# az16/MD_RDM

Measured on AMD Instinct MI355X. Metric: depth-maps/sec NYU 228x304 batch=16 fwd+bwd, higher is better.
Workload: dtype f32 (bf16x6-split 1x1 forward of dense_e2/e3, bf16x3-split gradient GEMMs of dense_e2/e3/e4); 1 GPU; NYU-v2 228x304 batch=16/GPU full train step (fwd+losses+bwd+AdamW), DepthEstimationNet 90.5M params; global_batch=16, parallelism=dp1

## Files before the change

### md_rdm_amd/csrc/xsplit.hip

```cpp
#include <algorithm>
#include <stdlib.h>

#include "rdm_common.h"
#include "elementwise.h"
#include "xsplit.h"
#include "xsplit_dev.h"

namespace rdm {

namespace {

__device__ __forceinline__ bf16x8 tr_frag(const unsigned char* base0, const unsigned char* base1, int imm) {
#if defined(__HIP_DEVICE_COMPILE__)
  typedef s16x4 __attribute__((address_space(3))) * lds_s16x4;
  const s16x4 a = __builtin_amdgcn_ds_read_tr16_b64_v4i16((lds_s16x4)(base0 + imm));
  const s16x4 b = __builtin_amdgcn_ds_read_tr16_b64_v4i16((lds_s16x4)(base1 + imm));
  const s16x8 ab = {a.x, a.y, a.z, a.w, b.x, b.y, b.z, b.w};
  return __builtin_bit_cast(bf16x8, ab);
#else
  return bf16x8{};
#endif
}

struct XsWgradArgs {
  const float* G; int ldg; int N;
  int g_bf16;
  int g_split, x_split;
  const float* X; int ldx; int C;
  const float* x_scale; const float* x_shift;
  float* dW; int ldw;
  int M, split_k;
  unsigned g_bytes, x_bytes;
  int n_ctiles;
  int ct_c0[12], ct_nt[12];
};

constexpr int XS_BM = 256, XS_BK = 32, XS_NTMAX = 12;
constexpr int XS_A_IMG = XS_BK * XS_BM * 2;
constexpr int XS_B_IMG = XS_BK * XS_NTMAX * 16 * 2;
constexpr int XS_STAGE = 2 * XS_A_IMG + 2 * XS_B_IMG;

template <int NT, int NP>
__device__ __forceinline__ void xs_wgrad1x1_body(const XsWgradArgs& p, unsigned char* smem, int c0, int n0, int s_begin, int s_end) {
  constexpr int BN = NT * 16;
  constexpr int TW = (NT + 1) / 2;
  constexpr int BPATCH = 8 * NT;
  constexpr int BL = (BPATCH + 31) / 32;
  float* const Ssc = reinterpret_cast<float*>(smem + 2 * XS_STAGE);

  const int tid = threadIdx.x, lane = tid & 63, wave = tid >> 6;
  const int wn = wave & 3, wc = wave >> 2;
  const int t0 = wc ? TW : 0, ntw = wc ? NT / 2 : TW;
  const int l16 = lane & 15, g = lane >> 4;
  const int grp = tid >> 4, kq = l16 >> 2, jq = l16 & 3;
  const bool bnrelu = p.x_scale != nullptr;
  const __amdgpu_buffer_rsrc_t srdG = make_srd(p.G, p.g_bytes), srdX = make_srd(p.X, p.x_bytes);

  if (bnrelu) {
    for (int i = tid; i < BN; i += 512) {
      const bool ok = c0 + i < p.C;
      Ssc[i] = ok ? p.x_scale[c0 + i] : 0.f;
      Ssc[BN + i] = ok ? p.x_shift[c0 + i] : 0.f;
    }
  }

  unsigned a_voff[4]; int a_row[4]; unsigned a_lds[4];
#pragma unroll
  for (int it = 0; it < 4; ++it) {
    const int rg = (grp >> 4) + 2 * it, ct = grp & 15;
    const int row = 4 * rg + kq, n = n0 + 16 * ct + 4 * jq;
    a_row[it] = n < p.N ? row : 0x40000000;
    a_voff[it] = (NP == 1 && p.g_bf16) ? (unsigned)row * (unsigned)(p.ldg * 2) + (unsigned)(n * 2) : (unsigned)row * (unsigned)(p.ldg * 4) + (unsigned)(n * 4);
    const int rb = row >> 3, pr = (row & 7) ^ ((rb & 1) << 2);
    a_lds[it] = (unsigned)(256 * (rb * 16 + ct) + 32 * pr + 8 * jq);
  }
  unsigned b_voff[BL]; int b_row[BL]; unsigned b_lds[BL]; int b_col[BL];
#pragma unroll
  for (int it = 0; it < BL; ++it) {
    const int pi = grp + 32 * it;
    const int rg = pi / NT, ct = pi - rg * NT;
    const int row = 4 * rg + kq, cl = 16 * ct + 4 * jq;
    const bool ok = pi < BPATCH && c0 + cl < p.C;
    b_row[it] = ok ? row : 0x40000000;
// ... 741 lines not shown
      bf16x8 ah[3], al[3];
#pragma unroll
      for (int nt = 0; nt < 3; ++nt) {
        ah[nt] = tr_frag(gb + frG0, gb + frG1, 256 * nt);
        al[nt] = tr_frag(gb + XW_GPLANE + frG0, gb + XW_GPLANE + frG1, 256 * nt);
      }
      const unsigned soff = ((unsigned)s * 4096u) & (unsigned)(XW_YPLANE - 1);
#pragma unroll
      for (int tap = 0; tap < 9; ++tap) {
        const bf16x8 bh = y_frag(Yhi, soff, tap), bl = y_frag(Ylo, soff, tap);
#pragma unroll
        for (int nt = 0; nt < 3; ++nt) {
          if (NP == 3) {
            acc[tap][nt] = __builtin_amdgcn_mfma_f32_16x16x32_bf16(al[nt], bh, acc[tap][nt], 0, 0, 0);
            acc[tap][nt] = __builtin_amdgcn_mfma_f32_16x16x32_bf16(ah[nt], bl, acc[tap][nt], 0, 0, 0);
          }
          acc[tap][nt] = __builtin_amdgcn_mfma_f32_16x16x32_bf16(ah[nt], bh, acc[tap][nt], 0, 0, 0);
        }
      }
      if (more) { store_y((u + 1) % XW_D, s + 1 + p.ahead); store_g((u + 1) % XW_D, s + 1); }
      __syncthreads();
    }
  }

  const int c = c0 + 16 * wave + l16;
#pragma unroll
  for (int tap = 0; tap < 9; ++tap)
#pragma unroll
    for (int nt = 0; nt < 3; ++nt)
#pragma unroll
      for (int r = 0; r < 4; ++r) {
        const int n = nt * 16 + 4 * g + r;
        if (c < p.C && n < p.N) atomicAdd(p.dW + (long)tap * p.wtap + (long)n * p.ldw + c, acc[tap][nt][r]);
      }
}


constexpr int XF_NTW = 6, XF_BNMAX = 2 * XF_NTW * 16;
constexpr int XF_W_IMG = XF_BNMAX * 64;
constexpr int xf_x_img(int mtw) { return 4 * mtw * 16 * 64; }
constexpr int xf_lds(int mtw) { return 3 * xf_x_img(mtw) + 3 * XF_W_IMG; }

struct XsFwd1Args {
  const float* X; int ldx; int K;
  const float* x_scale; const float* x_shift;
  const unsigned char* Wp;
  float* out; int ldc;
  double* stat0; double* stat1;
  int M, N, ksteps, PT, mtiles, ctiles;
  unsigned x_bytes, w_bytes;
};

__global__ __launch_bounds__(256) void k_xs_pack_w1_fwd(const float* __restrict__ w, int ldw, int N, int K, int ksteps, unsigned char* __restrict__ Wp) {
  const long idx = (long)blockIdx.x * 256 + threadIdx.x;
  const int ch = (int)(idx & 3);
  const long r1 = idx >> 2;
  const int n = (int)(r1 % N), j = (int)(r1 / N);
  if (j >= ksteps) return;
  f32x4 v0, v1;
#pragma unroll
  for (int e = 0; e < 4; ++e) {
    const int k0 = 32 * j + 8 * ch + e, k1 = k0 + 4;
    v0[e] = k0 < K ? w[(long)n * ldw + k0] : 0.f;
    v1[e] = k1 < K ? w[(long)n * ldw + k1] : 0.f;
  }
  u32x2 a0, a1, a2, b0, b1, b2;
  split3x4(v0[0], v0[1], v0[2], v0[3], a0, a1, a2);
  split3x4(v1[0], v1[1], v1[2], v1[3], b0, b1, b2);
  const int chs = ch ^ (((n >> 2) & 1) << 1);
  const long plane = (long)ksteps * N * 64;
  unsigned char* dst = Wp + ((long)j * N + n) * 64 + chs * 16;
  *reinterpret_cast<u32x4*>(dst) = u32x4{a0[0], a0[1], b0[0], b0[1]};
  *reinterpret_cast<u32x4*>(dst + plane) = u32x4{a1[0], a1[1], b1[0], b1[1]};
  *reinterpret_cast<u32x4*>(dst + 2 * plane) = u32x4{a2[0], a2[1], b2[0], b2[1]};
}

template <bool STATS, int NP, int MTW>
__global__ __launch_bounds__(512, MTW == 4 ? 2 : 4) void xs_fwd1x1_kernel(XsFwd1Args p) {
  constexpr int XF_MTW = MTW, XF_X_IMG = xf_x_img(MTW);
  extern __shared__ __attribute__((aligned(1024))) unsigned char xf_smem[];
  const int tid = threadIdx.x, lane = tid & 63, wave = __builtin_amdgcn_readfirstlane(tid >> 6);
  const int l16 = lane & 15, g = lane >> 4;
  const int wc = wave & 1, wp = wave >> 1;
  const unsigned total = gridDim.x, L = blockIdx.x, xq = L & 7u, qq = total >> 3, rr = total & 7u;
  const unsigned item = xq * qq + (xq < rr ? xq : rr) + (L >> 3);
  const int mt = (int)(item / (unsigned)p.ctiles), ctile = (int)(item - (unsigned)mt * (unsigned)p.ctiles);
  const int BM = p.PT * 16, m0 = mt * BM;
  const int ct0 = ctile * (2 * XF_NTW), nct = min(2 * XF_NTW, p.N / 16 - ct0), BN = nct * 16;
  const int ntw_max = (nct + 1) >> 1, tw0 = wc * ntw_max, ntw = min(ntw_max, nct - tw0);
  const int npw_max = (p.PT + 3) >> 2, pw0 = wp * npw_max, npw = max(0, min(npw_max, p.PT - pw0));
  const __amdgpu_buffer_rsrc_t srdX = make_srd(p.X, p.x_bytes), srdW = make_srd(p.Wp, p.w_bytes);
  const bool bnrelu = p.x_scale != nullptr;
  unsigned char* const Xi = xf_smem;
  unsigned char* const Wi = xf_smem + 3 * XF_X_IMG;

  unsigned x_voff[XF_MTW]; unsigned x_lds[XF_MTW]; bool x_ok[XF_MTW];
  const int f4 = tid & 7;
#pragma unroll
  for (int u = 0; u < XF_MTW; ++u) {
    const int row = (tid + 512 * u) >> 3;
    x_ok[u] = row < BM && m0 + row < p.M;
    x_voff[u] = (unsigned)(m0 + row) * (unsigned)(p.ldx * 4) + (unsigned)(f4 * 16);
    x_lds[u] = (unsigned)(row * 64 + (((f4 >> 1) ^ (((row >> 2) & 1) << 1)) * 16) + (f4 & 1) * 8);
  }
  const int wpieces = BN * 4;
  const unsigned w_plane = (unsigned)p.ksteps * (unsigned)p.N * 64u;
  f32x4 rx[XF_MTW], sc, sh; u32x4 rw[5];
  auto load_slab = [&](int j) {
    const bool kok = 32 * j + 4 * f4 < p.K;
#pragma unroll
    for (int u = 0; u < XF_MTW; ++u)
      rx[u] = __builtin_bit_cast(f32x4, __builtin_amdgcn_raw_buffer_load_b128(srdX, (int)((x_ok[u] && kok) ? x_voff[u] + (unsigned)(j * 128) : OOB), 0, 0));
    if (bnrelu) {
      sc = kok ? *reinterpret_cast<const f32x4*>(p.x_scale + 32 * j + 4 * f4) : f32x4{0.f, 0.f, 0.f, 0.f};
      sh = kok ? *reinterpret_cast<const f32x4*>(p.x_shift + 32 * j + 4 * f4) : f32x4{0.f, 0.f, 0.f, 0.f};
    }
#pragma unroll
    for (int u = 0; u < 5; ++u) {
      const int q = tid + 512 * u, pl = q / wpieces, r = q - pl * wpieces;
      rw[u] = __builtin_amdgcn_raw_buffer_load_b128(srdW, (int)(q < 3 * wpieces ? (unsigned)pl * w_plane + ((unsigned)j * (unsigned)p.N + (unsigned)(ct0 * 16)) * 64u + (unsigned)r * 16u : OOB), 0, 0);
    }
  };
  auto store_slab = [&]() {
#pragma unroll
    for (int u = 0; u < XF_MTW; ++u) {
      if ((tid + 512 * u) >> 3 < BM) {
        f32x4 v = rx[u];
        if (bnrelu) {
#pragma unroll
          for (int e = 0; e < 4; ++e) v[e] = fmaxf(fmaf(v[e], sc[e], sh[e]), 0.f);
        }
        u32x2 p0, p1, p2;
        split3x4(v[0], v[1], v[2], v[3], p0, p1, p2);
        *reinterpret_cast<u32x2*>(Xi + x_lds[u]) = p0;
        if (NP == 6) {
          *reinterpret_cast<u32x2*>(Xi + XF_X_IMG + x_lds[u]) = p1;
          *reinterpret_cast<u32x2*>(Xi + 2 * XF_X_IMG + x_lds[u]) = p2;
        }
      }
    }
#pragma unroll
    for (int u = 0; u < 5; ++u) {
      const int q = tid + 512 * u, pl = q / wpieces, r = q - pl * wpieces;
      if (q < 3 * wpieces) *reinterpret_cast<u32x4*>(Wi + pl * XF_W_IMG + r * 16) = rw[u];
    }
  };

  f32x4 acc[XF_MTW][XF_NTW];
#pragma unroll
  for (int i = 0; i < XF_MTW; ++i)
#pragma unroll
    for (int t = 0; t < XF_NTW; ++t) acc[i][t] = f32x4{0.f, 0.f, 0.f, 0.f};
  const unsigned fr = (unsigned)(l16 * 64 + ((g ^ (((l16 >> 2) & 1) << 1)) * 16));

  load_slab(0);
  for (int j = 0; j < p.ksteps; ++j) {
    store_slab();
    __syncthreads();
    if (j + 1 < p.ksteps) load_slab(j + 1);
    bf16x8 x0[XF_MTW], x1[XF_MTW], x2[XF_MTW];
#pragma unroll
    for (int i = 0; i < XF_MTW; ++i)
      if (i < npw) {
        x0[i] = *reinterpret_cast<const bf16x8*>(Xi + (pw0 + i) * 1024 + fr);
        x1[i] = *reinterpret_cast<const bf16x8*>(Xi + XF_X_IMG + (pw0 + i) * 1024 + fr);
        x2[i] = *reinterpret_cast<const bf16x8*>(Xi + 2 * XF_X_IMG + (pw0 + i) * 1024 + fr);
      }
#pragma unroll
    for (int t = 0; t < XF_NTW; ++t)
      if (t < ntw) {
        const bf16x8 w0 = *reinterpret_cast<const bf16x8*>(Wi + (tw0 + t) * 1024 + fr);
        const bf16x8 w1 = *reinterpret_cast<const bf16x8*>(Wi + XF_W_IMG + (tw0 + t) * 1024 + fr);
        const bf16x8 w2 = *reinterpret_cast<const bf16x8*>(Wi + 2 * XF_W_IMG + (tw0 + t) * 1024 + fr);
#pragma unroll
        for (int i = 0; i < XF_MTW; ++i)
          if (i < npw) {
            if (NP == 6) {
              acc[i][t] = __builtin_amdgcn_mfma_f32_16x16x32_bf16(w1, x1[i], acc[i][t], 0, 0, 0);
              acc[i][t] = __builtin_amdgcn_mfma_f32_16x16x32_bf16(w2, x0[i], acc[i][t], 0, 0, 0);
              acc[i][t] = __builtin_amdgcn_mfma_f32_16x16x32_bf16(w0, x2[i], acc[i][t], 0, 0, 0);
              acc[i][t] = __builtin_amdgcn_mfma_f32_16x16x32_bf16(w1, x0[i], acc[i][t], 0, 0, 0);
              acc[i][t] = __builtin_amdgcn_mfma_f32_16x16x32_bf16(w0, x1[i], acc[i][t], 0, 0, 0);
            }
            acc[i][t] = __builtin_amdgcn_mfma_f32_16x16x32_bf16(w0, x0[i], acc[i][t], 0, 0, 0);
          }
      }
    __syncthreads();
  }

#pragma unroll
  for (int t = 0; t < XF_NTW; ++t) {
    if (t >= ntw) continue;
    const int n4 = (ct0 + tw0 + t) * 16 + 4 * g;
    const bool nok = n4 < p.N;
    f32x4 s0 = {0.f, 0.f, 0.f, 0.f}, s1 = {0.f, 0.f, 0.f, 0.f};
#pragma unroll
    for (int i = 0; i < XF_MTW; ++i) {
      const int m = m0 + (pw0 + i) * 16 + l16;
      const bool ok = nok && i < npw && m < p.M;
      const f32x4 v = acc[i][t];
      if (ok) {
        *reinterpret_cast<f32x4*>(p.out + (long)m * p.ldc + n4) = v;
        if (STATS) { s0 += v; s1 += v * v; }
      }
    }
    if (STATS) {
#pragma unroll
      for (int e = 0; e < 4; ++e) {
        float a = s0[e], b = s1[e];
        a += __shfl_xor(a, 1); b += __shfl_xor(b, 1);
        a += __shfl_xor(a, 2); b += __shfl_xor(b, 2);
        a += __shfl_xor(a, 4); b += __shfl_xor(b, 4);
        a += __shfl_xor(a, 8); b += __shfl_xor(b, 8);
        if (l16 == e) { s0[0] = a; s1[0] = b; }
      }
      if (l16 < 4 && nok && npw > 0) {
        atomicAdd(p.stat0 + n4 + l16, (double)s0[0]);
        atomicAdd(p.stat1 + n4 + l16, (double)s1[0]);
      }
    }
  }
}

}

bool xs_wgrad1x1_supported(const WgradArgs& a) {
  const bool one = a.g.KH == 1 && a.g.KW == 1 && a.g.SH == 1 && a.g.SW == 1 && a.g.PH == 0 && a.g.PW == 0 && a.g.H == a.g.Ho && a.g.W == a.g.Wo;
  return one && a.C % 48 == 0 && a.C >= 96 && a.C <= 12 * 192 && a.N % 4 == 0;
}

int launch_xs_wgrad1x1(const WgradArgs& a, hipStream_t s) {
  RDM_CHECK_ARG(xs_wgrad1x1_supported(a), "split-precision 1x1 wgrad: needs a 1x1 / stride 1 convolution with 96 <= C (%d) <= 2304, C a multiple of 48, N (%d) of 4", a.C, a.N);
  RDM_CHECK_ARG(a.ldg % 4 == 0 && a.ldx % 4 == 0 && ((uintptr_t)a.G & 15) == 0 && ((uintptr_t)a.Xs & 15) == 0, "split-precision 1x1 wgrad: strides multiples of 4 floats, operands 16-byte aligned");
  const long M = (long)a.g.B * a.g.Ho * a.g.Wo;
  RDM_CHECK_ARG(!a.g_bf16 || a.xsplit == 1, "1x1 wgrad: bf16 gradient rows exist in the one-product (mixed-precision) form only");
  const long gb = ((M - 1) * a.ldg + a.N) * (a.g_bf16 ? 2 : 4), xb = ((M - 1) * a.ldx + a.C) * 4;
  if (gb >= 0xFFFFFFFFL || xb >= 0xFFFFFFFFL) { set_error("split-precision 1x1 wgrad: operand extent >= 4 GiB is not supported by the 32-bit buffer addressing"); return RDM_ERR_UNSUPPORTED; }
  RDM_CHECK_ARG((!a.g_split && !a.x_split) || a.xsplit != 1, "1x1 wgrad: split rows are operands of the three-product form");
  RDM_CHECK_ARG(!a.x_split || (a.x_scale == nullptr && a.x_shift == nullptr), "1x1 wgrad: split activation rows are already activated (no BatchNorm prologue)");
  XsWgradArgs k{};
  k.g_bf16 = a.g_bf16; k.g_split = a.g_split; k.x_split = a.x_split;
  k.G = a.G; k.ldg = a.ldg; k.N = a.N; k.X = a.Xs; k.ldx = a.ldx; k.C = a.C; k.x_scale = a.x_scale; k.x_shift = a.x_shift;
  k.dW = a.dW; k.ldw = a.ldw; k.M = (int)M; k.g_bytes = (unsigned)gb; k.x_bytes = (unsigned)xb;
  const int units = a.C / 48, nct = (units + 3) / 4;
  int c0 = 0;
  for (int t = 0; t < nct; ++t) {
    const int u = units / nct + (t < units % nct ? 1 : 0);
    k.ct_c0[t] = c0; k.ct_nt[t] = 3 * u;
    c0 += 48 * u;
  }
  k.n_ctiles = nct;
  const long tiles = (long)nct * cdiv(a.N, XS_BM), kslabs = (M + XS_BK - 1) / XS_BK;
  const long tiles128 = (long)nct * cdiv(a.N, 128);
  const long split128 = tiles128 > 512 ? pick_split_k(tiles128, kslabs / 2, 256 * 2) : std::max<long>(1, std::min<long>(512 / tiles128, kslabs / 16));
  long split = 1;
  if (split128 > 1) split = std::max<long>(2, tiles > 256 ? pick_split_k(tiles, kslabs / 2, 256) : std::min<long>(256 / tiles, kslabs / 16));
  if (a.split_k > 0) split = a.split_k;
  k.split_k = (int)std::min<long>(split, kslabs);
  void* prof = profile_begin(s, 2.0 * (double)M * a.N * a.C, 13);
  RDM_CENSUS("xs_wgrad1x1_kernel/x%d/%s/%s%s", a.xsplit == 1 ? 1 : 3, a.x_scale ? "bn1" : "bn0", k.split_k > 1 ? "splitK" : "split1", a.g_split && a.x_split ? "/rowsGX" : a.g_split ? "/rowsG" : a.x_split ? "/rowsX" : "");
  if (a.xsplit == 1) hipLaunchKernelGGL(xs_wgrad1x1_kernel<1>, dim3((unsigned)(tiles * k.split_k)), dim3(512), 0, s, k);
  else hipLaunchKernelGGL(xs_wgrad1x1_kernel<3>, dim3((unsigned)(tiles * k.split_k)), dim3(512), 0, s, k);
  profile_end(prof, s);
  RDM_LAUNCH_OK();
  return 0;
}

size_t xs_dgrad3x3_workspace_bytes(int Cb) { return (size_t)(Cb / 16) * XD_KSTEPS * 2048; }

static int xs_dgrad3_lds_bytes(int W) {
  const int nslots = 1 + XD_BM + 2 * (W + 1);
  const int plane = (nslots * XD_SLOT + 1023) & ~1023;
  return 2 * plane;
}

bool xs_dgrad3x3_supported(const FwdArgs& a) {
  const ConvGeom& g = a.g;
  return g.KH == 3 && g.KW == 3 && g.SH == 1 && g.SW == 1 && g.PH == 1 && g.PW == 1 && g.H == g.Ho && g.W == g.Wo && g.dir == -1 && a.C == 48 &&
         a.N % 16 == 0 && a.N >= 16 && xs_dgrad3_lds_bytes(g.W) <= 156 * 1024 && (g.W + 2) * XD_SLOT < 32768 && a.bias == nullptr && !a.accumulate && !a.add_out;
}

int launch_xs_pack_w3_dgrad(const float* w, long wtap, int ldw, int Cb, void* ws, hipStream_t s) {
  const long threads = (long)(Cb / 16) * XD_KSTEPS * 64;
  hipLaunchKernelGGL(k_xs_pack_w3_dgrad, dim3((unsigned)cdiv(threads, 256)), dim3(256), 0, s, w, wtap, ldw, Cb, static_cast<unsigned char*>(ws));
  RDM_LAUNCH_OK();
  return 0;
}

int launch_xs_dgrad3x3(const FwdArgs& a, Epilogue epi, void* ws, size_t ws_bytes, hipStream_t s, int np, bool prepacked) {
  RDM_CHECK_ARG(xs_dgrad3x3_supported(a), "split-precision 3x3 dgrad: needs a 3x3 / stride 1 / pad 1 convolution with 48 gradient channels, N (%d) a multiple of 16, W (%d) <= 339", a.N, a.g.W);
  RDM_CHECK_ARG(epi == EPI_STORE || epi == EPI_MASK_STATS, "split-precision 3x3 dgrad: plain or gate + statistics epilogue only");
  RDM_CHECK_ARG(a.lda % 4 == 0 && a.ldc % 4 == 0 && a.ldw % 4 == 0 && ((uintptr_t)a.A & 15) == 0 && ((uintptr_t)a.out & 15) == 0, "split-precision 3x3 dgrad: strides multiples of 4 floats, tensors 16-byte aligned");
  RDM_CHECK_ARG(epi != EPI_MASK_STATS || (a.X && a.x_scale && a.x_shift && a.stat0 && a.stat1 && a.ldx % 4 == 0 && ((uintptr_t)a.X & 15) == 0), "split-precision 3x3 dgrad: the gate needs X, scale, shift and both statistics");
  RDM_CHECK_ARG(ws != nullptr && ((uintptr_t)ws & 15) == 0 && ws_bytes >= xs_dgrad3x3_workspace_bytes(a.N), "split-precision 3x3 dgrad: workspace too small or misaligned (%zu < %zu)", ws_bytes, xs_dgrad3x3_workspace_bytes(a.N));
  const long M = a.M;
  const long gb = ((M - 1) * a.lda + 48) * 4, ob = ((M - 1) * a.ldc + a.N) * 4, xb = a.X ? ((M - 1) * a.ldx + a.N) * 4 : 16;
  if (gb >= 0xFFFFFFFFL || ob >= 0xFFFFFFFFL || xb >= 0xFFFFFFFFL) { set_error("split-precision 3x3 dgrad: operand extent >= 4 GiB is not supported by the 32-bit buffer addressing"); return RDM_ERR_UNSUPPORTED; }
  const int Cb = a.N;
  if (!prepacked) { if (int prc = launch_xs_pack_w3_dgrad(a.Wt, a.wtap, a.ldw, Cb, ws, s)) return prc; }
  XsDgrad3Args k{};
  k.G = a.A; k.ldg = a.lda; k.Wf = static_cast<const unsigned char*>(ws); k.out = a.out; k.ldc = a.ldc;
  k.X = a.X; k.ldx = a.ldx; k.x_scale = a.x_scale; k.x_shift = a.x_shift; k.stat0 = a.stat0; k.stat1 = a.stat1;
  RDM_CHECK_ARG(!a.out_bf16 || np == 1, "3x3 dgrad: bf16 output rows exist in the one-product (mixed-precision) form only");
// ... 85 lines not shown
  RDM_LAUNCH_OK();
  return 0;
}

__global__ __launch_bounds__(256) void k_frame_split_rows(const float* __restrict__ G, int ldg, int N, int B, int H, int W, int upad, u32x4* __restrict__ dst) {
  const int Wp = W + 2, PP = (H + 2) * Wp;
  const float rPP = 1.0f / (float)PP, rWp = 1.0f / (float)Wp;
  const int t = threadIdx.x, pl = (int)((unsigned)t * 2731u >> 15), q = t - pl * 12;
  if (t >= 252) return;
  for (int u = blockIdx.x * 21 + pl; u < upad; u += gridDim.x * 21) {
    const int b = (int)(((float)u + 0.5f) * rPP), rem = u - b * PP, yp = (int)(((float)rem + 0.5f) * rWp), xp = rem - yp * Wp;
    f32x4 v = {0.f, 0.f, 0.f, 0.f};
    if (b < B && yp >= 1 && yp <= H && xp >= 1 && xp <= W && 4 * q < N) v = *reinterpret_cast<const f32x4*>(G + ((long)(b * H + yp - 1) * W + xp - 1) * ldg + 4 * q);
    dst[(long)u * 12 + q] = split_row4(v[0], v[1], v[2], v[3]);
  }
}

size_t xs_frame_rows_bytes(int B, int H, int W) { return (size_t)(((long)B * (H + 2) * (W + 2) + 31) / 32 * 32) * 192; }

int launch_frame_split_rows(const float* G, int ldg, int N, int B, int H, int W, void* dst, hipStream_t s) {
  RDM_CHECK_ARG(N >= 4 && N <= 48 && N % 4 == 0 && ldg % 4 == 0 && ((uintptr_t)G & 15) == 0 && ((uintptr_t)dst & 15) == 0, "frame_split_rows: N (%d) a multiple of 4 up to 48, ldg a multiple of 4, operands 16-byte aligned", N);
  const long upad = ((long)B * (H + 2) * (W + 2) + 31) / 32 * 32;
  RDM_CHECK_ARG(upad < (1L << 21), "frame_split_rows: %ld padded positions (the float-reciprocal frame arithmetic is exact below 2^21)", upad);
  hipLaunchKernelGGL(k_frame_split_rows, dim3((unsigned)std::min<long>(cdiv(upad, 21), 256 * 16)), dim3(256), 0, s, G, ldg, N, B, H, W, (int)upad, static_cast<u32x4*>(dst));
  RDM_LAUNCH_OK();
  return 0;
}

bool xs_wgrad3x3_supported(const WgradArgs& a) {
  const ConvGeom& g = a.g;
  return g.KH == 3 && g.KW == 3 && g.SH == 1 && g.SW == 1 && g.PH == 1 && g.PW == 1 && g.H == g.Ho && g.W == g.Wo && g.dir == 1 && a.N <= 48 && a.N % 4 == 0 &&
         a.C % 4 == 0 && a.C >= 16 && (g.W + 3 + 31) / 32 <= 3;
}

int launch_xs_wgrad3x3(const WgradArgs& a, hipStream_t s) {
  RDM_CHECK_ARG(xs_wgrad3x3_supported(a), "split-precision 3x3 wgrad: needs a 3x3 / stride 1 / pad 1 convolution with N (%d) <= 48, N and C (%d) multiples of 4, W (%d) <= 93", a.N, a.C, a.g.W);
  RDM_CHECK_ARG(a.ldg % 4 == 0 && a.ldx % 4 == 0 && a.ldw % 4 == 0 && ((uintptr_t)a.G & 15) == 0 && ((uintptr_t)a.Xs & 15) == 0, "split-precision 3x3 wgrad: strides multiples of 4 floats, operands 16-byte aligned");
  const long M = (long)a.g.B * a.g.H * a.g.W;
  RDM_CHECK_ARG(!a.g_frame || a.xsplit != 1, "3x3 wgrad: the frame image is an operand of the three-product form");
  const long gb = a.g_frame ? (long)xs_frame_rows_bytes(a.g.B, a.g.H, a.g.W) : ((M - 1) * a.ldg + a.N) * 4, yb = ((M - 1) * a.ldx + a.C) * 4;
  if (gb >= 0xFFFFFFFFL || yb >= 0xFFFFFFFFL) { set_error("split-precision 3x3 wgrad: operand extent >= 4 GiB is not supported by the 32-bit buffer addressing"); return RDM_ERR_UNSUPPORTED; }
  XsWgrad3Args k{};
  k.g_frame = a.g_frame;
  k.G = a.G; k.ldg = a.ldg; k.Y = a.Xs; k.ldy = a.ldx; k.C = a.C; k.y_scale = a.x_scale; k.y_shift = a.x_shift;
  k.dW = a.dW; k.wtap = a.wtap; k.ldw = a.ldw; k.N = a.N; k.B = a.g.B; k.H = a.g.H; k.W = a.g.W;
  const long U = (long)a.g.B * (a.g.H + 2) * (a.g.W + 2);
  k.nslab = (int)((U + 31) / 32);
  k.ahead = (a.g.W + 3 + 31) / 32;
  const int cblocks = cdiv(a.C, XW_BC);
  int best = 1; double best_cost = 1e30;
  const int max_split = a.split_k > 0 ? a.split_k : 64;
  for (int sp = a.split_k > 0 ? a.split_k : 1; sp <= max_split && sp <= std::max(1, k.nslab / 8); ++sp) {
    const long rounds = ((long)cblocks * sp + 511) / 512;
    const double cost = rounds * ((k.nslab + sp - 1) / sp + 2.0 * k.ahead + 3.0 + 8.0);
    if (cost < best_cost - 1e-9) { best_cost = cost; best = sp; }
  }
  k.split = best;
  k.g_bytes = (unsigned)gb; k.y_bytes = (unsigned)yb;
  void* prof = profile_begin(s, 2.0 * (double)M * a.N * 9.0 * a.C, 15);
  RDM_CENSUS("xs_wgrad3x3_kernel/x%d/%s%s", a.xsplit == 1 ? 1 : 3, a.x_scale ? "bn1" : "bn0", a.g_frame ? "/frameG" : "");
  if (a.xsplit == 1) hipLaunchKernelGGL(xs_wgrad3x3_kernel<1>, dim3((unsigned)cblocks, (unsigned)k.split), dim3(256), 0, s, k);
  else hipLaunchKernelGGL(xs_wgrad3x3_kernel<3>, dim3((unsigned)cblocks, (unsigned)k.split), dim3(256), 0, s, k);
  profile_end(prof, s);
  RDM_LAUNCH_OK();
  return 0;
}

size_t xs_fwd1x1_workspace_bytes(int K, int N) { return (size_t)3 * ((K + 31) / 32) * N * 64; }

bool xs_fwd1x1_supported(const FwdArgs& a) {
  const ConvGeom& g = a.g;
  const bool one = g.KH == 1 && g.KW == 1 && g.SH == 1 && g.SW == 1 && g.PH == 0 && g.PW == 0 && g.H == g.Ho && g.W == g.Wo && g.dir == 1;
  return one && a.N % 16 == 0 && a.N >= 16 && a.C % 4 == 0 && a.C >= 4 && a.bias == nullptr && !a.accumulate && !a.add_out && a.a_sum == nullptr;
}

int launch_xs_pack_w1_fwd(const float* w, int ldw, int N, int K, void* ws, hipStream_t s) {
  const int ksteps = (K + 31) / 32;
  const long threads = (long)ksteps * N * 4;
  hipLaunchKernelGGL(k_xs_pack_w1_fwd, dim3((unsigned)cdiv(threads, 256)), dim3(256), 0, s, w, ldw, N, K, ksteps, static_cast<unsigned char*>(ws));
  RDM_LAUNCH_OK();
  return 0;
}

int launch_xs_fwd1x1(const FwdArgs& a, Epilogue epi, void* ws, size_t ws_bytes, hipStream_t s, int np, bool prepacked) {
  RDM_CHECK_ARG(xs_fwd1x1_supported(a), "split-precision 1x1 forward: needs a 1x1 / stride 1 convolution, N (%d) a multiple of 16, C (%d) a multiple of 4, no bias / accumulation", a.N, a.C);
  RDM_CHECK_ARG(epi == EPI_STORE || epi == EPI_STORE_STATS, "split-precision 1x1 forward: plain or statistics epilogue only");
  RDM_CHECK_ARG(a.lda % 4 == 0 && a.ldc % 4 == 0 && a.ldw % 4 == 0 && ((uintptr_t)a.A & 15) == 0 && ((uintptr_t)a.out & 15) == 0, "split-precision 1x1 forward: strides multiples of 4 floats, tensors 16-byte aligned");
  RDM_CHECK_ARG((a.a_scale == nullptr) == (a.a_shift == nullptr) && (a.a_scale == nullptr || (((uintptr_t)a.a_scale | (uintptr_t)a.a_shift) & 15) == 0), "split-precision 1x1 forward: scale and shift go together, 16-byte aligned");
  RDM_CHECK_ARG(epi != EPI_STORE_STATS || (a.stat0 && a.stat1), "split-precision 1x1 forward: the statistics epilogue needs both sums");
  const int K = a.C, N = a.N, ksteps = (K + 31) / 32;
  RDM_CHECK_ARG(ws != nullptr && ((uintptr_t)ws & 15) == 0 && ws_bytes >= xs_fwd1x1_workspace_bytes(K, N), "split-precision 1x1 forward: workspace too small or misaligned (%zu < %zu)", ws_bytes, xs_fwd1x1_workspace_bytes(K, N));
  const long M = a.M;
  const long xb = ((M - 1) * a.lda + K) * 4;
  if (xb >= 0xFFFFFFFFL) { set_error("split-precision 1x1 forward: operand extent >= 4 GiB is not supported by the 32-bit buffer addressing"); return RDM_ERR_UNSUPPORTED; }
  if (!prepacked) { if (int prc = launch_xs_pack_w1_fwd(a.Wt, a.ldw, N, K, ws, s)) return prc; }
  XsFwd1Args k{};
  k.X = a.A; k.ldx = a.lda; k.K = K; k.x_scale = a.a_scale; k.x_shift = a.a_shift; k.Wp = static_cast<const unsigned char*>(ws);
  k.out = a.out; k.ldc = a.ldc; k.stat0 = a.stat0; k.stat1 = a.stat1; k.M = (int)M; k.N = N; k.ksteps = ksteps;
  k.ctiles = cdiv(N / 16, 2 * XF_NTW);
  constexpr int mtw = 4, slots = 256;
  int best_pt = 1; long best_cost = -1;
  for (int pt = 1; pt <= 4 * mtw; ++pt) {
    const long items = (long)cdiv(M, 16 * pt) * k.ctiles, rounds = (items + slots - 1) / slots;
    const long cost = rounds * (pt * 16 + 24);
    if (best_cost < 0 || cost < best_cost) { best_cost = cost; best_pt = pt; }
  }
  k.PT = best_pt; k.mtiles = cdiv(M, 16 * best_pt);
  k.x_bytes = (unsigned)xb; k.w_bytes = (unsigned)xs_fwd1x1_workspace_bytes(K, N);
  void* prof = profile_begin(s, 2.0 * (double)M * N * K, 17);
  RDM_CENSUS("xs_fwd1x1_kernel/x%d/%s/%s", np == 1 ? 1 : 6, a.a_scale ? "bn1" : "bn0", epi == EPI_STORE_STATS ? "STORE_STATS" : "STORE");
  const dim3 grid((unsigned)(k.mtiles * k.ctiles));
#define RDM_XS_F1M(STATS_, NP_, MTW_) do { \
    RDM_HIP_OK(hipFuncSetAttribute(reinterpret_cast<const void*>(&xs_fwd1x1_kernel<STATS_, NP_, MTW_>), hipFuncAttributeMaxDynamicSharedMemorySize, xf_lds(MTW_))); \
    hipLaunchKernelGGL((xs_fwd1x1_kernel<STATS_, NP_, MTW_>), grid, dim3(512), xf_lds(MTW_), s, k); } while (0)
#define RDM_XS_F1(STATS_, NP_) RDM_XS_F1M(STATS_, NP_, 4)
  if (epi == EPI_STORE_STATS) { if (np == 1) RDM_XS_F1(true, 1); else RDM_XS_F1(true, 6); }
  else { if (np == 1) RDM_XS_F1(false, 1); else RDM_XS_F1(false, 6); }
#undef RDM_XS_F1
#undef RDM_XS_F1M
  profile_end(prof, s);
  RDM_LAUNCH_OK();
  return 0;
}

}
```

Before: 343.8 images/s.

## Make split-precision 1x1 forward kernel persistent with cross-tile prefetch

```diff
diff --git a/md_rdm_amd/csrc/xsplit.hip b/md_rdm_amd/csrc/xsplit.hip
--- a/md_rdm_amd/csrc/xsplit.hip
+++ b/md_rdm_amd/csrc/xsplit.hip
@@ -1,4 +1,5 @@
 #include <algorithm>
+#include <atomic>
 #include <stdlib.h>
 
 #include "rdm_common.h"
@@ -906,35 +907,44 @@
   const int tid = threadIdx.x, lane = tid & 63, wave = __builtin_amdgcn_readfirstlane(tid >> 6);
   const int l16 = lane & 15, g = lane >> 4;
   const int wc = wave & 1, wp = wave >> 1;
-  const unsigned total = gridDim.x, L = blockIdx.x, xq = L & 7u, qq = total >> 3, rr = total & 7u;
-  const unsigned item = xq * qq + (xq < rr ? xq : rr) + (L >> 3);
-  const int mt = (int)(item / (unsigned)p.ctiles), ctile = (int)(item - (unsigned)mt * (unsigned)p.ctiles);
-  const int BM = p.PT * 16, m0 = mt * BM;
-  const int ct0 = ctile * (2 * XF_NTW), nct = min(2 * XF_NTW, p.N / 16 - ct0), BN = nct * 16;
-  const int ntw_max = (nct + 1) >> 1, tw0 = wc * ntw_max, ntw = min(ntw_max, nct - tw0);
+  const unsigned G = gridDim.x, L = blockIdx.x, xq = L & 7u, qq = G >> 3, rr = G & 7u;
+  const unsigned wg = xq * qq + (xq < rr ? xq : rr) + (L >> 3);
+  const long T = (long)p.mtiles * p.ctiles;
+  const int it0 = (int)((long)wg * T / G), it1 = (int)((long)(wg + 1) * T / G);
+  if (it0 >= it1) return;
+  const int BM = p.PT * 16;
   const int npw_max = (p.PT + 3) >> 2, pw0 = wp * npw_max, npw = max(0, min(npw_max, p.PT - pw0));
   const __amdgpu_buffer_rsrc_t srdX = make_srd(p.X, p.x_bytes), srdW = make_srd(p.Wp, p.w_bytes);
   const bool bnrelu = p.x_scale != nullptr;
   unsigned char* const Xi = xf_smem;
   unsigned char* const Wi = xf_smem + 3 * XF_X_IMG;
 
-  unsigned x_voff[XF_MTW]; unsigned x_lds[XF_MTW]; bool x_ok[XF_MTW];
+  struct Item { int m0, ct0, nct; };
+  auto decode = [&](int it) {
+    const int mt = (int)((unsigned)it / (unsigned)p.ctiles), ctile = it - mt * p.ctiles;
+    Item r;
+    r.m0 = mt * BM; r.ct0 = ctile * (2 * XF_NTW); r.nct = min(2 * XF_NTW, p.N / 16 - r.ct0);
+    return r;
+  };
+
+  unsigned x_voff[XF_MTW]; unsigned x_lds[XF_MTW];
   const int f4 = tid & 7;
 #pragma unroll
   for (int u = 0; u < XF_MTW; ++u) {
     const int row = (tid + 512 * u) >> 3;
-    x_ok[u] = row < BM && m0 + row < p.M;
-    x_voff[u] = (unsigned)(m0 + row) * (unsigned)(p.ldx * 4) + (unsigned)(f4 * 16);
+    x_voff[u] = (unsigned)row * (unsigned)(p.ldx * 4) + (unsigned)(f4 * 16);
     x_lds[u] = (unsigned)(row * 64 + (((f4 >> 1) ^ (((row >> 2) & 1) << 1)) * 16) + (f4 & 1) * 8);
   }
-  const int wpieces = BN * 4;
   const unsigned w_plane = (unsigned)p.ksteps * (unsigned)p.N * 64u;
   f32x4 rx[XF_MTW], sc, sh; u32x4 rw[5];
-  auto load_slab = [&](int j) {
+  auto load_slab = [&](const Item& I, int j) {
     const bool kok = 32 * j + 4 * f4 < p.K;
+    const int rows = min(BM, p.M - I.m0);
+    const unsigned xb = (unsigned)I.m0 * (unsigned)(p.ldx * 4) + (unsigned)(j * 128);
+    const int wpieces = I.nct * 64;
 #pragma unroll
     for (int u = 0; u < XF_MTW; ++u)
-      rx[u] = __builtin_bit_cast(f32x4, __builtin_amdgcn_raw_buffer_load_b128(srdX, (int)((x_ok[u] && kok) ? x_voff[u] + (unsigned)(j * 128) : OOB), 0, 0));
+      rx[u] = __builtin_bit_cast(f32x4, __builtin_amdgcn_raw_buffer_load_b128(srdX, (int)((((tid + 512 * u) >> 3) < rows && kok) ? x_voff[u] + xb : OOB), 0, 0));
     if (bnrelu) {
       sc = kok ? *reinterpret_cast<const f32x4*>(p.x_scale + 32 * j + 4 * f4) : f32x4{0.f, 0.f, 0.f, 0.f};
       sh = kok ? *reinterpret_cast<const f32x4*>(p.x_shift + 32 * j + 4 * f4) : f32x4{0.f, 0.f, 0.f, 0.f};
@@ -942,10 +952,11 @@
 #pragma unroll
     for (int u = 0; u < 5; ++u) {
       const int q = tid + 512 * u, pl = q / wpieces, r = q - pl * wpieces;
-      rw[u] = __builtin_amdgcn_raw_buffer_load_b128(srdW, (int)(q < 3 * wpieces ? (unsigned)pl * w_plane + ((unsigned)j * (unsigned)p.N + (unsigned)(ct0 * 16)) * 64u + (unsigned)r * 16u : OOB), 0, 0);
+      rw[u] = __builtin_amdgcn_raw_buffer_load_b128(srdW, (int)(q < 3 * wpieces ? (unsigned)pl * w_plane + ((unsigned)j * (unsigned)p.N + (unsigned)(I.ct0 * 16)) * 64u + (unsigned)r * 16u : OOB), 0, 0);
     }
   };
-  auto store_slab = [&]() {
+  auto store_slab = [&](const Item& I) {
+    const int wpieces = I.nct * 64;
 #pragma unroll
     for (int u = 0; u < XF_MTW; ++u) {
       if ((tid + 512 * u) >> 3 < BM) {
@@ -977,72 +988,82 @@
     for (int t = 0; t < XF_NTW; ++t) acc[i][t] = f32x4{0.f, 0.f, 0.f, 0.f};
   const unsigned fr = (unsigned)(l16 * 64 + ((g ^ (((l16 >> 2) & 1) << 1)) * 16));
 
-  load_slab(0);
-  for (int j = 0; j < p.ksteps; ++j) {
-    store_slab();
-    __syncthreads();
-    if (j + 1 < p.ksteps) load_slab(j + 1);
-    bf16x8 x0[XF_MTW], x1[XF_MTW], x2[XF_MTW];
+  Item cur = decode(it0);
+  load_slab(cur, 0);
+  for (int it = it0; it < it1; ++it) {
+    const int m0 = cur.m0, ct0 = cur.ct0, nct = cur.nct;
+    const int ntw_max = (nct + 1) >> 1, tw0 = wc * ntw_max, ntw = min(ntw_max, nct - tw0);
+    for (int j = 0; j < p.ksteps; ++j) {
+      store_slab(cur);
+      __syncthreads();
+      if (j + 1 < p.ksteps) load_slab(cur, j + 1);
+      bf16x8 x0[XF_MTW], x1[XF_MTW], x2[XF_MTW];
+#pragma unroll
+      for (int i = 0; i < XF_MTW; ++i)
+        if (i < npw) {
+          x0[i] = *reinterpret_cast<const bf16x8*>(Xi + (pw0 + i) * 1024 + fr);
+          x1[i] = *reinterpret_cast<const bf16x8*>(Xi + XF_X_IMG + (pw0 + i) * 1024 + fr);
+          x2[i] = *reinterpret_cast<const bf16x8*>(Xi + 2 * XF_X_IMG + (pw0 + i) * 1024 + fr);
+        }
+#pragma unroll
+      for (int t = 0; t < XF_NTW; ++t)
+        if (t < ntw) {
+          const bf16x8 w0 = *reinterpret_cast<const bf16x8*>(Wi + (tw0 + t) * 1024 + fr);
+          const bf16x8 w1 = *reinterpret_cast<const bf16x8*>(Wi + XF_W_IMG + (tw0 + t) * 1024 + fr);
+          const bf16x8 w2 = *reinterpret_cast<const bf16x8*>(Wi + 2 * XF_W_IMG + (tw0 + t) * 1024 + fr);
+#pragma unroll
+          for (int i = 0; i < XF_MTW; ++i)
+            if (i < npw) {
+              if (NP == 6) {
+                acc[i][t] = __builtin_amdgcn_mfma_f32_16x16x32_bf16(w1, x1[i], acc[i][t], 0, 0, 0);
+                acc[i][t] = __builtin_amdgcn_mfma_f32_16x16x32_bf16(w2, x0[i], acc[i][t], 0, 0, 0);
+                acc[i][t] = __builtin_amdgcn_mfma_f32_16x16x32_bf16(w0, x2[i], acc[i][t], 0, 0, 0);
+                acc[i][t] = __builtin_amdgcn_mfma_f32_16x16x32_bf16(w1, x0[i], acc[i][t], 0, 0, 0);
+                acc[i][t] = __builtin_amdgcn_mfma_f32_16x16x32_bf16(w0, x1[i], acc[i][t], 0, 0, 0);
+              }
+              acc[i][t] = __builtin_amdgcn_mfma_f32_16x16x32_bf16(w0, x0[i], acc[i][t], 0, 0, 0);
+            }
+        }
+      __syncthreads();
+    }
+    if (it + 1 < it1) { cur = decode(it + 1); load_slab(cur, 0); }
+
+#pragma unroll
+    for (int t = 0; t < XF_NTW; ++t) {
+      if (t >= ntw) continue;
+      const int n4 = (ct0 + tw0 + t) * 16 + 4 * g;
+      const bool nok = n4 < p.N;
+      f32x4 s0 = {0.f, 0.f, 0.f, 0.f}, s1 = {0.f, 0.f, 0.f, 0.f};
+#pragma unroll
+      for (int i = 0; i < XF_MTW; ++i) {
+        const int m = m0 + (pw0 + i) * 16 + l16;
+        const bool ok = nok && i < npw && m < p.M;
+        const f32x4 v = acc[i][t];
+        if (ok) {
+          *reinterpret_cast<f32x4*>(p.out + (long)m * p.ldc + n4) = v;
+          if (STATS) { s0 += v; s1 += v * v; }
+        }
+      }
+      if (STATS) {
+#pragma unroll
+        for (int e = 0; e < 4; ++e) {
+          float a = s0[e], b = s1[e];
+          a += __shfl_xor(a, 1); b += __shfl_xor(b, 1);
+          a += __shfl_xor(a, 2); b += __shfl_xor(b, 2);
+          a += __shfl_xor(a, 4); b += __shfl_xor(b, 4);
+          a += __shfl_xor(a, 8); b += __shfl_xor(b, 8);
+          if (l16 == e) { s0[0] = a; s1[0] = b; }
+        }
+        if (l16 < 4 && nok && npw > 0) {
+          atomicAdd(p.stat0 + n4 + l16, (double)s0[0]);
+          atomicAdd(p.stat1 + n4 + l16, (double)s1[0]);
+        }
+      }
+    }
 #pragma unroll
     for (int i = 0; i < XF_MTW; ++i)
-      if (i < npw) {
-        x0[i] = *reinterpret_cast<const bf16x8*>(Xi + (pw0 + i) * 1024 + fr);
-        x1[i] = *reinterpret_cast<const bf16x8*>(Xi + XF_X_IMG + (pw0 + i) * 1024 + fr);
-        x2[i] = *reinterpret_cast<const bf16x8*>(Xi + 2 * XF_X_IMG + (pw0 + i) * 1024 + fr);
-      }
-#pragma unroll
-    for (int t = 0; t < XF_NTW; ++t)
-      if (t < ntw) {
-        const bf16x8 w0 = *reinterpret_cast<const bf16x8*>(Wi + (tw0 + t) * 1024 + fr);
-        const bf16x8 w1 = *reinterpret_cast<const bf16x8*>(Wi + XF_W_IMG + (tw0 + t) * 1024 + fr);
-        const bf16x8 w2 = *reinterpret_cast<const bf16x8*>(Wi + 2 * XF_W_IMG + (tw0 + t) * 1024 + fr);
-#pragma unroll
-        for (int i = 0; i < XF_MTW; ++i)
-          if (i < npw) {
-            if (NP == 6) {
-              acc[i][t] = __builtin_amdgcn_mfma_f32_16x16x32_bf16(w1, x1[i], acc[i][t], 0, 0, 0);
-              acc[i][t] = __builtin_amdgcn_mfma_f32_16x16x32_bf16(w2, x0[i], acc[i][t], 0, 0, 0);
-              acc[i][t] = __builtin_amdgcn_mfma_f32_16x16x32_bf16(w0, x2[i], acc[i][t], 0, 0, 0);
-              acc[i][t] = __builtin_amdgcn_mfma_f32_16x16x32_bf16(w1, x0[i], acc[i][t], 0, 0, 0);
-              acc[i][t] = __builtin_amdgcn_mfma_f32_16x16x32_bf16(w0, x1[i], acc[i][t], 0, 0, 0);
-            }
-            acc[i][t] = __builtin_amdgcn_mfma_f32_16x16x32_bf16(w0, x0[i], acc[i][t], 0, 0, 0);
-          }
-      }
-    __syncthreads();
-  }
-
-#pragma unroll
-  for (int t = 0; t < XF_NTW; ++t) {
-    if (t >= ntw) continue;
-    const int n4 = (ct0 + tw0 + t) * 16 + 4 * g;
-    const bool nok = n4 < p.N;
-    f32x4 s0 = {0.f, 0.f, 0.f, 0.f}, s1 = {0.f, 0.f, 0.f, 0.f};
-#pragma unroll
-    for (int i = 0; i < XF_MTW; ++i) {
-      const int m = m0 + (pw0 + i) * 16 + l16;
-      const bool ok = nok && i < npw && m < p.M;
-      const f32x4 v = acc[i][t];
-      if (ok) {
-        *reinterpret_cast<f32x4*>(p.out + (long)m * p.ldc + n4) = v;
-        if (STATS) { s0 += v; s1 += v * v; }
-      }
-    }
-    if (STATS) {
-#pragma unroll
-      for (int e = 0; e < 4; ++e) {
-        float a = s0[e], b = s1[e];
-        a += __shfl_xor(a, 1); b += __shfl_xor(b, 1);
-        a += __shfl_xor(a, 2); b += __shfl_xor(b, 2);
-        a += __shfl_xor(a, 4); b += __shfl_xor(b, 4);
-        a += __shfl_xor(a, 8); b += __shfl_xor(b, 8);
-        if (l16 == e) { s0[0] = a; s1[0] = b; }
-      }
-      if (l16 < 4 && nok && npw > 0) {
-        atomicAdd(p.stat0 + n4 + l16, (double)s0[0]);
-        atomicAdd(p.stat1 + n4 + l16, (double)s1[0]);
-      }
-    }
+#pragma unroll
+      for (int t = 0; t < XF_NTW; ++t) acc[i][t] = f32x4{0.f, 0.f, 0.f, 0.f};
   }
 }
 
@@ -1294,6 +1315,26 @@
   return 0;
 }
 
+template <bool STATS, int NP, int MTW>
+static int xf_launch(const XsFwd1Args& k, long items, hipStream_t s) {
+  const void* fn = reinterpret_cast<const void*>(&xs_fwd1x1_kernel<STATS, NP, MTW>);
+  RDM_HIP_OK(hipFuncSetAttribute(fn, hipFuncAttributeMaxDynamicSharedMemorySize, xf_lds(MTW)));
+  static std::atomic<int> resident[16];
+  int dev = 0;
+  RDM_HIP_OK(hipGetDevice(&dev));
+  int slots = resident[dev & 15].load(std::memory_order_relaxed);
+  if (slots == 0) {
+    int per_cu = 0, cus = 0;
+    RDM_HIP_OK(hipOccupancyMaxActiveBlocksPerMultiprocessor(&per_cu, fn, 512, xf_lds(MTW)));
+    RDM_HIP_OK(hipDeviceGetAttribute(&cus, hipDeviceAttributeMultiprocessorCount, dev));
+    RDM_CHECK_ARG(per_cu > 0 && cus > 0, "split-precision 1x1 forward: not launchable on this device (%d workgroups per CU, %d CUs)", per_cu, cus);
+    slots = per_cu * cus;
+    resident[dev & 15].store(slots, std::memory_order_relaxed);
+  }
+  hipLaunchKernelGGL((xs_fwd1x1_kernel<STATS, NP, MTW>), dim3((unsigned)std::min<long>(items, slots)), dim3(512), xf_lds(MTW), s, k);
+  return 0;
+}
+
 int launch_xs_fwd1x1(const FwdArgs& a, Epilogue epi, void* ws, size_t ws_bytes, hipStream_t s, int np, bool prepacked) {
   RDM_CHECK_ARG(xs_fwd1x1_supported(a), "split-precision 1x1 forward: needs a 1x1 / stride 1 convolution, N (%d) a multiple of 16, C (%d) a multiple of 4, no bias / accumulation", a.N, a.C);
   RDM_CHECK_ARG(epi == EPI_STORE || epi == EPI_STORE_STATS, "split-precision 1x1 forward: plain or statistics epilogue only");
@@ -1321,15 +1362,11 @@
   k.x_bytes = (unsigned)xb; k.w_bytes = (unsigned)xs_fwd1x1_workspace_bytes(K, N);
   void* prof = profile_begin(s, 2.0 * (double)M * N * K, 17);
   RDM_CENSUS("xs_fwd1x1_kernel/x%d/%s/%s", np == 1 ? 1 : 6, a.a_scale ? "bn1" : "bn0", epi == EPI_STORE_STATS ? "STORE_STATS" : "STORE");
-  const dim3 grid((unsigned)(k.mtiles * k.ctiles));
-#define RDM_XS_F1M(STATS_, NP_, MTW_) do { \
-    RDM_HIP_OK(hipFuncSetAttribute(reinterpret_cast<const void*>(&xs_fwd1x1_kernel<STATS_, NP_, MTW_>), hipFuncAttributeMaxDynamicSharedMemorySize, xf_lds(MTW_))); \
-    hipLaunchKernelGGL((xs_fwd1x1_kernel<STATS_, NP_, MTW_>), grid, dim3(512), xf_lds(MTW_), s, k); } while (0)
-#define RDM_XS_F1(STATS_, NP_) RDM_XS_F1M(STATS_, NP_, 4)
-  if (epi == EPI_STORE_STATS) { if (np == 1) RDM_XS_F1(true, 1); else RDM_XS_F1(true, 6); }
-  else { if (np == 1) RDM_XS_F1(false, 1); else RDM_XS_F1(false, 6); }
-#undef RDM_XS_F1
-#undef RDM_XS_F1M
+  const long items = (long)k.mtiles * k.ctiles;
+  int rc;
+  if (epi == EPI_STORE_STATS) rc = np == 1 ? xf_launch<true, 1, 4>(k, items, s) : xf_launch<true, 6, 4>(k, items, s);
+  else rc = np == 1 ? xf_launch<false, 1, 4>(k, items, s) : xf_launch<false, 6, 4>(k, items, s);
+  if (rc) return rc;
   profile_end(prof, s);
   RDM_LAUNCH_OK();
   return 0;
```

Result: no change. 345.6 images/s, median of 6 (+0.5%).
